# kogdenko/con-gen

Measured on AMD Instinct MI355X. Metric: Gpkts/s + GB/s device-resident checksum, 64B & 1500B batches; %HBM peak, higher is better.
Workload: dtype u16; 1 GPU; 16777216 x 1500 B IPv4+TCP per GPU, dense stride 1500, ip_cksum + tcp_cksum per packet (BASELINE configs[2]; configs[4] at 8 GPUs); packets_per_gpu=16777216, packet_bytes=1500, parallelism=batch-split x1

## Files before the change

### con-gen_amd/csrc/cgck_lane.hip

```cpp
#include "cgck_lane.h"

#include <stdlib.h>
#include <optional>

namespace cgck {


template <bool DESC, bool NT, int S0, bool CLAMP>
__global__ __launch_bounds__(256) void lpp_kernel(KParams p)
{
	const bool raw = p.flags & CGCK_RAW;
	const Sched sc = sched((p.n + 255) / 256, p.contig);
	for (uint64_t it = sc.it; it < sc.end; it += sc.step) {
		const uint64_t k = it * 256 + threadIdx.x;
		const Pkt pk = get_pkt<DESC>(p, k);
		const uint64_t a0 = pk.a0;
		const int len = (int)pk.len, q = (int)(a0 & 15), nch = nchunks(a0, pk.len);
		const uint4 *c0 = reinterpret_cast<const uint4 *>(a0 & ~(uint64_t)15);
		uint4 v[S0];
#pragma unroll
		for (int i = 0; i < S0; ++i)
			v[i] = CLAMP ? ldc<NT>(c0, i, nch, p.zero) : (i < nch ? ld<NT>(c0 + i) : make_uint4(0, 0, 0, 0));
		const bool more = __any(nch > S0);
		uint4 last = make_uint4(0, 0, 0, 0);
		if (CLAMP) {
			if (more)
				last = ldc<NT>(c0, nch - 1, nch, p.zero);
		} else {
			last = nch > S0 ? ld<NT>(c0 + nch - 1) : make_uint4(0, 0, 0, 0);
		}

		uint32_t tot = 0;
#pragma unroll
		for (int i = 0; i < S0; ++i)
			tot = i < nch ? sum4(v[i], tot) : tot;
		Hdr h{};
		if (!raw)
			h = header<S0, NT>(v, c0, nch, q, len, p.flags, pk.ok);
		if (more) {
			for (int t = S0; __any(t < nch - 1); t += 8) {
				uint4 w[8];
#pragma unroll
				for (int i = 0; i < 8; ++i)
					w[i] = t + i < nch - 1 ? ld<NT>(c0 + t + i) : make_uint4(0, 0, 0, 0);
				uint32_t s = 0;
#pragma unroll
				for (int i = 0; i < 8; ++i)
					s = sum4(w[i], s);
				tot = fold16(tot) + fold16(s);
			}
		}
		const bool dw = !__any(((q | len) & 3) != 0);
		if (__any(q != 0))
			tot = fold16(tot) + (0xffffu - fold16(lead_sum(v[0], q, dw)));
		const int e = q + len - 16 * (nch - 1);
		if (more)
			tot = fold16(tot) + fold16(nch > S0 ? sum4(last, 0) - trail_sum(last, e, dw) : 0u);
		if (__any(nch > 0 && nch <= S0 && e != 16)) {
			uint4 lc = make_uint4(0, 0, 0, 0);
#pragma unroll
			for (int i = 0; i < S0; ++i)
				if (i == nch - 1)
					lc = v[i];
			tot = fold16(tot) + (0xffffu - fold16(nch > 0 && nch <= S0 ? trail_sum(lc, e, dw) : 0u));
		}
		if (pk.ok)
			finish(p, k, a0, len, fold16(tot), h);
	}
}

struct Quad {
	uint4 c[4];
};

template <bool NT>
__device__ __forceinline__ void lpa_load(const KParams &p, uint64_t k, bool live, int nch, Quad &q)
{
	k = k < p.n ? k : p.n - 1;
	const uint4 *c0 = live ? reinterpret_cast<const uint4 *>(p.base + k * p.stride + p.l3_off)
			       : reinterpret_cast<const uint4 *>((const uint8_t *)p.zero + (blockIdx.x & 63) * 64);
#pragma unroll
	for (int i = 0; i < 4; ++i)
		q.c[i] = ld<NT>(c0 + (i < nch ? i : nch - 1));
}

template <bool NT, bool STAGE = false, bool IP6 = false>
__device__ __forceinline__ void lpa_reduce(const KParams &p, uint64_t k, int len, int nch, const Quad &q,
					   uint32_t *so = nullptr)
{
	const bool ok = k < p.n;
	if constexpr (IP6) {
		uint32_t T = 0;
#pragma unroll
		for (int i = 0; i < 4; ++i) {
			if (i < nch - 1 || (i == nch - 1 && (len & 15) == 0))
				T = sum4(q.c[i], T);
			else if (i == nch - 1)
				T = msum(q.c[i], 0, 0, len - 16 * i, T);
		}
		const uint32_t h8 = fold16(hsum(q.c[0].y, hsum(q.c[0].x, 0))), nh0 = (q.c[0].y >> 16) & 0xffu;
		const bool plain = len >= 40 && !__any(ok && (v6_is_ext(nh0) || nh0 == 44));
		if (ok) {
			const uint64_t a0 = reinterpret_cast<uint64_t>(p.base) + k * p.stride + p.l3_off;
			uint32_t bl = 0, out = 0;
			if (plain) {
				const int fo = v6_field(nh0);
				if (!(p.flags & CGCK_L4)) {
				} else if (fo >= 0 && 40 + fo + 2 > len) {
					bl = CGCK_BAD_LEN;
				} else {
					const uint32_t L = fold16(ocsub(fold16(T), h8) + (nh0 << 8) + bswap16((uint32_t)(len - 40)));
					out = finish(L) << 16;
				}
			} else {
				out = v6_dense(a0, len, fold16(T), h8, nh0, p.flags, &bl);
			}
			if (STAGE) {
				*so = out;
			} else if (p.out) {
				uint32_t *o = p.out + k;
				asm volatile("global_store_dword %0, %1, off nt" ::"v"(o), "v"(out) : "memory");
			}
			if (p.verdict)
				gbl(p.verdict)[k] = (uint8_t)bl;
		}
		return;
	}
	if (p.flags == (CGCK_IP | CGCK_L4) && (len & 15) == 0 && !__any(ok && (q.c[0].x & 15u) != 5u)) {
		uint32_t T = 0;
#pragma unroll
		for (int i = 0; i < 4; ++i)
			if (i < nch)
				T = sum4(q.c[i], T);
		const uint32_t IPs = fold16(hsum(q.c[1].x, sum4(q.c[0], 0)));
		const uint32_t PS = fold16(hsum(q.c[1].x, hsum(q.c[0].w, 0)));
		const uint32_t proto = (q.c[0].z >> 8) & 0xffu;
		uint32_t L = ocsub(fold16(T), IPs);
		L = fold16(L + PS + (proto << 8) + bswap16((uint32_t)(len - 20)));
		if (ok) {
			const uint32_t out = finish(IPs) | (finish(L) << 16);
			if (STAGE) {
				*so = out;
			} else if (p.out) {
				uint32_t *o = p.out + k;
				asm volatile("global_store_dword %0, %1, off nt" ::"v"(o), "v"(out) : "memory");
			}
			if (p.verdict)
				gbl(p.verdict)[k] = 0;
		}
		return;
	}
	uint4 v[6];
	v[4] = v[5] = make_uint4(0, 0, 0, 0);
#pragma unroll
	for (int i = 0; i < 4; ++i) {
		const int r1 = i < nch - 1 ? 16 : (i == nch - 1 ? len - 16 * i : 0);
		v[i] = make_uint4(q.c[i].x & dmask(0, 0, 0, r1), q.c[i].y & dmask(0, 1, 0, r1),
				  q.c[i].z & dmask(0, 2, 0, r1), q.c[i].w & dmask(0, 3, 0, r1));
	}
	uint32_t tot = 0;
#pragma unroll
	for (int i = 0; i < 4; ++i)
		tot = sum4(v[i], tot);
	const uint64_t a0 = reinterpret_cast<uint64_t>(p.base) + (ok ? k : 0) * p.stride + p.l3_off;
	Hdr h{};
	if (!(p.flags & CGCK_RAW))
		h = header<6, NT>(v, reinterpret_cast<const uint4 *>(a0), nch, 0, len, p.flags, ok);
	if (ok) {
		const Res r = result(p, a0, len, fold16(tot), h);
		if (p.out) {
			if (STAGE) {
				*so = r.out;
			} else {
				uint32_t *o = p.out + k;
				asm volatile("global_store_dword %0, %1, off nt" ::"v"(o), "v"(r.out) : "memory");
			}
		}
		if (p.verdict)
			gbl(p.verdict)[k] = (uint8_t)r.verdict;
	}
}

#define CGCK_LPA_KERNEL lpa_kernel
#define CGCK_LPD_KERNEL lpd_kernel
#define CGCK_LANE_IP6 false
#include "cgck_lane_kernels.inc"
#undef CGCK_LPA_KERNEL
#undef CGCK_LPD_KERNEL
#undef CGCK_LANE_IP6
#define CGCK_LPA_KERNEL lpa6_kernel
#define CGCK_LPD_KERNEL lpd6_kernel
#define CGCK_LANE_IP6 true
#include "cgck_lane_kernels.inc"
#undef CGCK_LPA_KERNEL
#undef CGCK_LPD_KERNEL
#undef CGCK_LANE_IP6


struct SMap {
	uint64_t a0;
	int len, nch;
	int s;
	int st, ns;
	int owner;
	int m;
	bool act;
};

template <bool DESC>
__device__ __forceinline__ SMap smap(const KParams &p, uint64_t cur, uint64_t r1, const DescW &d,
				     uint32_t (&mark)[64])
{
	const int l = threadIdx.x & 63;
	const Pkt pk = decode<DESC>(p, cur + l, r1, d);
	const int nch_l = nchunks(pk.a0, pk.len);
	const uint32_t ns = pk.ok ? (uint32_t)max(1, (nch_l + 7) >> 3) : 0u;
	const uint32_t P = wave_scan_dpp(ns);
	const uint64_t fit = __ballot(pk.ok && P <= 64);
	SMap M;
	M.m = __popcll(fit);
	const int T = M.m ? (int)__builtin_amdgcn_readlane(P, M.m - 1) : 0;
	mark[l] = 0;
	__builtin_amdgcn_wave_barrier();
	asm volatile("" ::: "memory");
	if (l < M.m)
		mark[P - ns] = 1;
	__builtin_amdgcn_wave_barrier();
	asm volatile("" ::: "memory");
	const uint64_t heads = __ballot(mark[l] != 0 && l < T);
	const uint64_t le = l == 63 ? ~0ull : ((2ull << l) - 1);
	const uint64_t below = heads & le, above = heads & ~le;
	M.act = l < T;
	M.owner = below ? __popcll(below) - 1 : 0;
	M.st = below ? 63 - __clzll(below) : 0;
	M.ns = (above ? __ffsll((long long)above) - 1 : T) - M.st;
	M.s = l - M.st;
	M.a0 = shfl64(pk.a0, M.owner);
	M.len = __shfl((int)pk.len, M.owner, 64);
	M.nch = nchunks(M.a0, (uint32_t)M.len);
	return M;
}

template <bool NT>
__device__ __forceinline__ void slot_issue(const KParams &p, const SMap &M, uint4 (&w)[8])
{
	const uint4 *c0 = reinterpret_cast<const uint4 *>(M.a0 & ~(uint64_t)15);
#pragma unroll
	for (int i = 0; i < 8; ++i)
		w[i] = ldc<NT>(c0, 8 * M.s + i, M.nch, p.zero);
}

template <bool NT>
__device__ __forceinline__ void slot_reduce(const KParams &p, uint64_t cur, const SMap &M, uint4 (&w)[8],
					    WaveStage &ws)
{
	const int l = threadIdx.x & 63;
	const bool raw = p.flags & CGCK_RAW;
	const uint64_t a0 = M.a0;
	const int len = M.len, nch = M.nch, s = M.s;
	const int q = (int)(a0 & 15);
	const uint4 *c0 = reinterpret_cast<const uint4 *>(a0 & ~(uint64_t)15);
#pragma unroll
	for (int i = 0; i < 8; ++i)
		asm volatile("" ::"v"(w[i].x), "v"(w[i].y), "v"(w[i].z), "v"(w[i].w));
	if (M.m == 0) {
		const int nsj = (nch + 7) >> 3;
		uint32_t acc = 0;
		Hdr h{};
		for (int wbase = 0; wbase < nsj; wbase += 64) {
			const int sj = wbase + l;
			uint4 (&v)[8] = w;
#pragma unroll
			for (int i = 0; i < 8; ++i)
				v[i] = ldc<NT>(c0, 8 * sj + i, nch, p.zero);
			uint32_t r = 0;
#pragma unroll
			for (int i = 0; i < 8; ++i)
				r = 8 * sj + i < nch ? sum4(v[i], r) : r;
			if (wbase == 0 && !raw)
				h = header<8, NT>(v, c0, nch, q, len, p.flags, l == 0);
			const int j = (nch - 1) - 8 * sj;
			const int e = q + len - 16 * (nch - 1);
			uint32_t corr = 0;
			if (sj == 0 && q != 0)
				corr += lead_sum(v[0], q, false);
			if (j >= 0 && j < 8 && e != 16)
				corr += trail_sum(pick8(v, j), e, false);
			r = fold16(r) + (0xffffu - fold16(corr));
			acc = fold16(acc) + fold16(gsum<64>(r));
		}
		wave_stage_reserve(p, ws, cur, 1);
		if (l == 0)
			wave_stage_put(ws, cur, result(p, a0, len, fold16(acc), h));
		__builtin_amdgcn_s_waitcnt(0);
		return;
	}
	const bool act = M.act;
	uint32_t r = 0;
#pragma unroll
	for (int i = 0; i < 8; ++i)
		r = act && 8 * s + i < nch ? sum4(w[i], r) : r;
	const bool head = act && s == 0;
	Hdr h{};
	if (!raw)
		h = header<8, NT>(w, c0, nch, q, len, p.flags, head);
	const bool dw = !__any(act && ((q | len) & 3) != 0);
	uint32_t corr = 0;
	if (__any(head && q != 0))
		corr = head && q != 0 ? lead_sum(w[0], q, dw) : 0u;
	const int j = (nch - 1) - 8 * s;
	const int e = q + len - 16 * (nch - 1);
	const bool tail = act && nch > 0 && j >= 0 && j < 8 && e != 16;
	if (__any(tail))
		corr += tail ? trail_sum(pick8(w, j), e, dw) : 0u;
	r = fold16(r) + (0xffffu - fold16(corr));
	uint32_t nso = 0;
#pragma unroll
	for (int b = 0; b < 7; ++b)
		nso |= __any(act && ((M.ns >> b) & 1)) ? (1u << b) : 0u;
	const int send = M.st + M.ns;
#pragma unroll
	for (int d = 1; d < 64; d <<= 1) {
		if ((uint32_t)d >= nso)
			break;
		const uint32_t y = __shfl_down(r, d, 64);
		if (l + d < send)
			r += y;
	}
	wave_stage_reserve(p, ws, cur, M.m);
	if (head)
		wave_stage_put(ws, cur + M.owner, result(p, a0, len, fold16(r), h));
}

#if !CGCK_LAB || !defined(CGCK_SLOT2_CHUNK)
#undef CGCK_SLOT2_CHUNK
#define CGCK_SLOT2_CHUNK 0
#endif
template <bool DESC, bool NT>
__global__ __launch_bounds__(256) void slot2_kernel(KParams p)
{
	__shared__ uint32_t mark[4][64];
	__shared__ uint32_t so[4][kWaveStage];
	__shared__ uint8_t sv[4][kWaveStage];
	const int wv = __builtin_amdgcn_readfirstlane(threadIdx.x >> 6), l = threadIdx.x & 63;
	const uint64_t nwaves = (uint64_t)gridDim.x * 4;
	const uint64_t wid = (uint64_t)blockIdx.x * 4 + wv;
#if CGCK_SLOT2_CHUNK
	for (uint64_t ck = wid; ck * CGCK_SLOT2_CHUNK < p.n; ck += nwaves) {
	const uint64_t r0 = ck * CGCK_SLOT2_CHUNK;
	const uint64_t r1 = r0 + CGCK_SLOT2_CHUNK < p.n ? r0 + CGCK_SLOT2_CHUNK : p.n;
#else
	const uint64_t per = (p.n + nwaves - 1) / nwaves;
	const uint64_t r0 = wid * per;
	const uint64_t r1 = r0 + per < p.n ? r0 + per : p.n;
	if (r0 >= r1)
		return;
#endif
	WaveStage ws{so[wv], sv[wv], r0};

	uint64_t curA = r0;
	SMap mA = smap<DESC>(p, curA, r1, load_desc<DESC>(p, curA + l, r1), mark[wv]);
	uint64_t curB = curA + (mA.m ? mA.m : 1);
	DescW dB = load_desc<DESC>(p, curB + l, r1);
	uint4 wA[8], wB[8];
	slot_issue<NT>(p, mA, wA);
	for (;;) {
		const SMap mB = smap<DESC>(p, curB, r1, dB, mark[wv]);
		const uint64_t curC = curB + (mB.m ? mB.m : 1);
		const DescW dC = load_desc<DESC>(p, curC + l, r1);
		slot_issue<NT>(p, mB, wB);
		slot_reduce<NT>(p, curA, mA, wA, ws);
		if (curB >= r1)
			break;
		const SMap mC = smap<DESC>(p, curC, r1, dC, mark[wv]);
		const uint64_t curD = curC + (mC.m ? mC.m : 1);
		dB = load_desc<DESC>(p, curD + l, r1);
		slot_issue<NT>(p, mC, wA);
		slot_reduce<NT>(p, curB, mB, wB, ws);
		if (curC >= r1)
			break;
		curA = curC;
		mA = mC;
		curB = curD;
	}
	wave_stage_flush(p, ws, r1);
#if CGCK_SLOT2_CHUNK
	}
#endif
}

#define CGCK_LPW_KERNEL lpw_kernel
#define CGCK_LPW_IP6 false
#define CGCK_LPW_FILL false
#define CGCK_LPW_MIXED false
#include "cgck_lpw_kernel.inc"
#undef CGCK_LPW_KERNEL
#undef CGCK_LPW_IP6
#undef CGCK_LPW_FILL
#undef CGCK_LPW_MIXED


template <bool DESC, int S0, bool CLAMP>
static hipError_t launch_lpp_t(const KParams &p, int max_blocks, bool nt, hipStream_t st)
{
	const unsigned blocks = grid_blocks(p.n, 256, max_blocks);
	if (nt) {
		CGCK_NOTE_KERNEL("lpp_kernel<%s, true, %d, %s>", tf(DESC), S0, tf(CLAMP));
		hipLaunchKernelGGL((lpp_kernel<DESC, true, S0, CLAMP>), dim3(blocks), dim3(256), 0, st, p);
	} else {
		CGCK_NOTE_KERNEL("lpp_kernel<%s, false, %d, %s>", tf(DESC), S0, tf(CLAMP));
		hipLaunchKernelGGL((lpp_kernel<DESC, false, S0, CLAMP>), dim3(blocks), dim3(256), 0, st, p);
	}
	return hipGetLastError();
}

#if CGCK_LAB
#include "cgck_lane_lab.inc"
#endif

hipError_t launch_lpp(const KParams &p, int num_cus, bool nt, int shape, hipStream_t st)
{
	const int mb = num_cus * 8;
#if CGCK_LAB
	if (const auto lab = launch_lpp_lab(p, mb, nt, shape, st))
		return *lab;
#endif
	return p.desc ? launch_lpp_t<true, 6, false>(p, mb, nt, st) : launch_lpp_t<false, 6, false>(p, mb, nt, st);
}

hipError_t launch_lpd(const KParams &p, int num_cus, hipStream_t st)
{
	static const int wpc = [] {
		const char *e = CGCK_ENV("CGCK_LPD_WPC");
		return e && atoi(e) > 0 ? atoi(e) : 8;
	}();
	const dim3 g(grid_blocks(p.n, 64 * 16, (uint64_t)num_cus * wpc));
	if (p.flags & CGCK_IP6) {
		CGCK_NOTE_KERNEL("lpd6_kernel<2, 32, 2>");
		hipLaunchKernelGGL((lpd6_kernel<2, 32, 2>), g, dim3(64), 2 * 4096 + 32 * 256, st, p);
		return hipGetLastError();
	}
#if CGCK_LAB
	if (const auto lab = launch_lpd_lab(p, g, num_cus, st))
		return *lab;
#endif
	CGCK_NOTE_KERNEL("lpd_kernel<2, 32, 2>");
	hipLaunchKernelGGL((lpd_kernel<2, 32, 2>), g, dim3(64), 2 * 4096 + 32 * 256, st, p);
	return hipGetLastError();
}

hipError_t launch_lpa(const KParams &p, int num_cus, bool nt, hipStream_t st)
{
	static const int bpc = [] {
		const char *e = CGCK_ENV("CGCK_LPA_BPC");
		return e && atoi(e) > 0 ? atoi(e) : 1;
	}();
	static const int depth = [] {
		const char *e = CGCK_ENV("CGCK_LPA_DEPTH");
		const int d = e ? atoi(e) : 0;
		return d >= 2 && d <= 4 ? d : 4;
	}();
	uint64_t want = (p.n + 255) / 256, mb = (uint64_t)num_cus * bpc;
	const dim3 g((unsigned)(want < mb ? want : mb));
	if (p.flags & CGCK_IP6) {
		if (nt) {
			CGCK_NOTE_KERNEL("lpa6_kernel<true, 4>");
			hipLaunchKernelGGL((lpa6_kernel<true, 4>), g, dim3(256), 0, st, p);
		} else {
			CGCK_NOTE_KERNEL("lpa6_kernel<false, 4>");
			hipLaunchKernelGGL((lpa6_kernel<false, 4>), g, dim3(256), 0, st, p);
		}
		return hipGetLastError();
	}
#define CGCK_LPA(D)                                                                            \
	do {                                                                                   \
		if (nt) {                                                                      \
			CGCK_NOTE_KERNEL("lpa_kernel<true, %d>", D);                           \
			hipLaunchKernelGGL((lpa_kernel<true, D>), g, dim3(256), 0, st, p);      \
		} else {                                                                       \
			CGCK_NOTE_KERNEL("lpa_kernel<false, %d>", D);                          \
			hipLaunchKernelGGL((lpa_kernel<false, D>), g, dim3(256), 0, st, p);     \
		}                                                                              \
	} while (0)
	if (depth == 4)
		CGCK_LPA(4);
	else if (depth == 3)
		CGCK_LPA(3);
	else
		CGCK_LPA(2);
#undef CGCK_LPA
	return hipGetLastError();
}

template <bool DESC>
static hipError_t launch_slot2_t(const KParams &p, int max_blocks, bool nt, hipStream_t st)
{
	const unsigned blocks = grid_blocks(p.n, 4 * 64, max_blocks);
	if (nt) {
		CGCK_NOTE_KERNEL("slot2_kernel<%s, true>", tf(DESC));
		hipLaunchKernelGGL((slot2_kernel<DESC, true>), dim3(blocks), dim3(256), 0, st, p);
	} else {
		CGCK_NOTE_KERNEL("slot2_kernel<%s, false>", tf(DESC));
		hipLaunchKernelGGL((slot2_kernel<DESC, false>), dim3(blocks), dim3(256), 0, st, p);
	}
	return hipGetLastError();
}

hipError_t launch_slot2(const KParams &p, int num_cus, bool nt, hipStream_t st)
{
	static const int bpc = [] {
		const char *e = CGCK_ENV("CGCK_BPC");
		return e && atoi(e) > 0 ? atoi(e) : 8;
	}();
	const int mb = num_cus * bpc;
	return p.desc ? launch_slot2_t<true>(p, mb, nt, st) : launch_slot2_t<false>(p, mb, nt, st);
}

hipError_t launch_lpw(const KParams &p, int num_cus, hipStream_t st)
{
	static const int wpc = [] {
		const char *e = CGCK_ENV("CGCK_LPW_WPC");
		return e && atoi(e) > 0 ? atoi(e) : 8;
	}();
	KParams q = p;
	q.contig = 0;
	const LpwShape sh = lpw_shape(p, num_cus, wpc, kLpwSlot);
#if CGCK_LAB
	if (const auto lab = launch_lpw_lab(p, q, sh.grid, sh.lds, num_cus, wpc, st))
		return *lab;
#endif
	if (p.desc) {
		CGCK_NOTE_KERNEL("lpw_kernel<true, %d, false>", kLpwC);
		hipLaunchKernelGGL((lpw_kernel<true, kLpwC, false>), sh.grid, dim3(64), sh.lds, st, q);
	} else {
		CGCK_NOTE_KERNEL("lpw_kernel<false, %d, false>", kLpwC);
		hipLaunchKernelGGL((lpw_kernel<false, kLpwC, false>), sh.grid, dim3(64), sh.lds, st, q);
	}
	return hipGetLastError();
}

}
```

### con-gen_amd/csrc/cgck_lane_kernels.inc

```
template <bool NT, int DEPTH>
__global__ __launch_bounds__(256) void CGCK_LPA_KERNEL(KParams p)
{
	constexpr bool IP6 = CGCK_LANE_IP6;
	const int len = (int)p.ip_len, nch = (len + 15) >> 4;
	const uint64_t NI = (p.n + 255) / 256, S = gridDim.x;
	uint64_t it = blockIdx.x;
	if (it >= NI)
		return;
	Quad Q[DEPTH];
#pragma unroll
	for (int d = 0; d < DEPTH - 1; ++d)
		lpa_load<NT>(p, (it + d * S) * 256 + threadIdx.x, it + d * S < NI, nch, Q[d]);
	for (;;) {
#pragma unroll
		for (int d = 0; d < DEPTH; ++d) {
			const uint64_t ahead = it + (uint64_t)(d + DEPTH - 1) * S;
			lpa_load<NT>(p, ahead * 256 + threadIdx.x, ahead < NI, nch, Q[(d + DEPTH - 1) % DEPTH]);
			lpa_reduce<NT, false, IP6>(p, (it + d * S) * 256 + threadIdx.x, len, nch, Q[d]);
			if (it + (uint64_t)(d + 1) * S >= NI)
				return;
		}
		it += (uint64_t)DEPTH * S;
	}
}

template <int D, int C, int SP>
__global__ __launch_bounds__(64) void CGCK_LPD_KERNEL(KParams p)
{
	constexpr bool IP6 = CGCK_LANE_IP6;
	extern __shared__ __attribute__((aligned(16))) uint8_t smem[];
	const int lane = threadIdx.x;
	const int len = (int)p.ip_len, nch = (len + 15) >> 4;
	const uint32_t lds0 = __builtin_amdgcn_readfirstlane((uint32_t)(uintptr_t)smem);
	uint32_t *so = reinterpret_cast<uint32_t *>(smem + D * 4096);
	const uint8_t *zero = (const uint8_t *)p.zero + (blockIdx.x & 63) * 64;
	const uint64_t base = reinterpret_cast<uint64_t>(p.base) + p.l3_off;
	const uint64_t last_chunk = (base + (p.n - 1) * p.stride + len - 1) & ~(uint64_t)15;
	const uint64_t NS = (p.n + 63) / 64, NC = (NS + C - 1) / C, G = gridDim.x, b = blockIdx.x;
	if (b >= NC)
		return;
	const uint64_t nsteps = (NC - b + G - 1) / G * C;
	auto gstep = [&](uint64_t j) { return (b + (j / C) * G) * C + j % C; };
	const uint32_t span = (uint32_t)(63 * p.stride) + (uint32_t)len;
	auto issue = [&](uint64_t j) {
		const uint64_t gs = gstep(j);
		const uint64_t a = base + gs * 64 * p.stride;
		const uint32_t slot = lds0 + (uint32_t)(j % D) * 4096;
#pragma unroll
		for (int i = 0; i < 4; ++i) {
			const uint32_t at = 1024 * i + 16 * lane;
			const uint64_t src = a + at;
			glds16_nt(j < nsteps && gs < NS && at < span && src <= last_chunk ? reinterpret_cast<const void *>(src)
											  : zero,
				  slot + 1024 * i);
		}
	};
#pragma unroll
	for (int d = 0; d < D - 1; ++d)
		issue(d);
	const int o = lane * (int)p.stride;
	constexpr bool stage = C > 1;
	constexpr bool DEFER = SP >= 3 && C > 1;
	constexpr int policy = SP % 3 == 0 ? kNt : SP % 3 == 1 ? kDefaultPolicy : kSc1;
	u32x4_t held[DEFER ? C / 4 : 1];
	bool pend = false;
	uint64_t pfirst = 0;
	for (uint64_t j = 0; j < nsteps; ++j) {
		issue(j + D - 1);
		if (DEFER && pend) {
			const __amdgpu_buffer_rsrc_t rs = out_rsrc(p.out + pfirst, C * 256);
#pragma unroll
			for (int i = 0; i < (DEFER ? C / 4 : 0); ++i)
				bstore16<policy>(rs, 16 * (i * 64 + lane), held[i]);
			pend = false;
		}
		if (C == 1) {
			if (j + 1 < (uint64_t)D || !p.out)
				asm volatile("s_waitcnt vmcnt(%0)" ::"i"(4 * (D - 1)) : "memory");
			else
				asm volatile("s_waitcnt vmcnt(%0)" ::"i"(5 * (D - 1)) : "memory");
		} else {
			if (stage && j >= (uint64_t)C && (j % C) <= (uint64_t)(DEFER ? D - 1 : D - 2))
				asm volatile("s_waitcnt vmcnt(%0)" ::"i"(4 * (D - 1) + C / 4) : "memory");
			else
				asm volatile("s_waitcnt vmcnt(%0)" ::"i"(4 * (D - 1)) : "memory");
		}
		__builtin_amdgcn_s_barrier();
		const uint8_t *sl = smem + (uint32_t)(j % D) * 4096;
		Quad q;
#pragma unroll
		for (int i = 0; i < 4; ++i)
			q.c[i] = *reinterpret_cast<const uint4 *>(sl + o + 16 * (i < nch ? i : nch - 1));
		asm volatile("s_waitcnt lgkmcnt(0)" ::: "memory");
		const uint64_t k = gstep(j) * 64 + lane;
		if (stage)
			lpa_reduce<false, true, IP6>(p, k, len, nch, q, so + (j % C) * 64 + lane);
		else
			lpa_reduce<false, false, IP6>(p, k, len, nch, q);
		if (stage && (j + 1) % C == 0 && p.contig != 2) {
			const uint64_t first = (b + (j / C) * G) * C * 64;
			asm volatile("s_waitcnt lgkmcnt(0)" ::: "memory");
			if (DEFER && first + C * 64 <= p.n && j + 1 < nsteps) {
				const u32x4_t *s4 = reinterpret_cast<const u32x4_t *>(so);
#pragma unroll
				for (int i = 0; i < (DEFER ? C / 4 : 0); ++i)
					held[i] = s4[i * 64 + lane];
				asm volatile("s_waitcnt lgkmcnt(0)" ::: "memory");
				pend = true;
				pfirst = first;
			} else if (first + C * 64 <= p.n) {
				const uint4 *s4 = reinterpret_cast<const uint4 *>(so);
				const __amdgpu_buffer_rsrc_t rs = out_rsrc(p.out + first, C * 256);
#pragma unroll
				for (int i = 0; i < C / 4; ++i) {
					const uint4 w = s4[i * 64 + lane];
					bstore16<policy>(rs, 16 * (i * 64 + lane), u32x4_t{w.x, w.y, w.z, w.w});
				}
			} else {
				for (int i = lane; i < C * 64; i += 64)
					if (first + i < p.n)
						gbl(p.out)[first + i] = so[i];
				asm volatile("s_waitcnt vmcnt(0)" ::: "memory");
			}
		}
	}
	asm volatile("s_waitcnt vmcnt(0)" ::: "memory");
}
```

Before: 4.523 Gpkt/s.

## Add specialized hot loop to LDS-staged checksum kernel with inline-asm batched loads

Splits the LPD kernel main loop into a hot phase covering full, in-bounds steps and a generic tail phase. The hot phase uses compile-time window counts and a fast-path flag, strength-reduced address and packet-index counters, and a single inline-asm block that issues the four global_load_lds_dwordx4 through m0 increments. It also precomputes LDS read indices and makes bounds checks unnecessary via a FULL template flag. The aim is to cut per-step scalar and vector ALU overhead (divisions, bounds checks, address math) so the kernel stays bandwidth-bound, at the cost of more code variants and fragile hand-written asm.

Measured after the change: 4.521 Gpkt/s. Within noise of the previous version (-0.1%).

```diff
diff --git a/con-gen_amd/csrc/cgck_lane.hip b/con-gen_amd/csrc/cgck_lane.hip
--- a/con-gen_amd/csrc/cgck_lane.hip
+++ b/con-gen_amd/csrc/cgck_lane.hip
@@ -84,11 +84,11 @@
 		q.c[i] = ld<NT>(c0 + (i < nch ? i : nch - 1));
 }
 
-template <bool NT, bool STAGE = false, bool IP6 = false>
+template <bool NT, bool STAGE = false, bool IP6 = false, int FAST = -1, bool FULL = false>
 __device__ __forceinline__ void lpa_reduce(const KParams &p, uint64_t k, int len, int nch, const Quad &q,
-					   uint32_t *so = nullptr)
-{
-	const bool ok = k < p.n;
+					   uint32_t *so = nullptr, uint64_t a0full = 0)
+{
+	const bool ok = FULL || k < p.n;
 	if constexpr (IP6) {
 		uint32_t T = 0;
 #pragma unroll
@@ -101,7 +101,7 @@
 		const uint32_t h8 = fold16(hsum(q.c[0].y, hsum(q.c[0].x, 0))), nh0 = (q.c[0].y >> 16) & 0xffu;
 		const bool plain = len >= 40 && !__any(ok && (v6_is_ext(nh0) || nh0 == 44));
 		if (ok) {
-			const uint64_t a0 = reinterpret_cast<uint64_t>(p.base) + k * p.stride + p.l3_off;
+			const uint64_t a0 = FULL ? a0full : reinterpret_cast<uint64_t>(p.base) + k * p.stride + p.l3_off;
 			uint32_t bl = 0, out = 0;
 			if (plain) {
 				const int fo = v6_field(nh0);
@@ -126,12 +126,13 @@
 		}
 		return;
 	}
-	if (p.flags == (CGCK_IP | CGCK_L4) && (len & 15) == 0 && !__any(ok && (q.c[0].x & 15u) != 5u)) {
+	if (FAST != 0 && (FAST == 1 || (p.flags == (CGCK_IP | CGCK_L4) && (len & 15) == 0)) &&
+	    !__any(ok && (q.c[0].x & 15u) != 5u)) {
 		uint32_t T = 0;
 #pragma unroll
 		for (int i = 0; i < 4; ++i)
 			if (i < nch)
-				T = sum4(q.c[i], T);
+				T += sum4(q.c[i], 0);
 		const uint32_t IPs = fold16(hsum(q.c[1].x, sum4(q.c[0], 0)));
 		const uint32_t PS = fold16(hsum(q.c[1].x, hsum(q.c[0].w, 0)));
 		const uint32_t proto = (q.c[0].z >> 8) & 0xffu;
@@ -162,7 +163,7 @@
 #pragma unroll
 	for (int i = 0; i < 4; ++i)
 		tot = sum4(v[i], tot);
-	const uint64_t a0 = reinterpret_cast<uint64_t>(p.base) + (ok ? k : 0) * p.stride + p.l3_off;
+	const uint64_t a0 = FULL ? a0full : reinterpret_cast<uint64_t>(p.base) + (ok ? k : 0) * p.stride + p.l3_off;
 	Hdr h{};
 	if (!(p.flags & CGCK_RAW))
 		h = header<6, NT>(v, reinterpret_cast<const uint4 *>(a0), nch, 0, len, p.flags, ok);
@@ -180,6 +181,45 @@
 			gbl(p.verdict)[k] = (uint8_t)r.verdict;
 	}
 }
+
+#define CGCK_LP_OPEN "s_mov_b32 %[k], m0\n\ts_mov_b32 m0, %[slot]\n\ts_nop 2\n\t"
+#define CGCK_LP_NEXT "s_add_u32 m0, m0, 0x400\n\ts_nop 0\n\t"
+#define CGCK_LP_W(i) "global_load_lds_dwordx4 %[o" #i "], %[a] nt\n\t"
+#define CGCK_LP_P "global_load_lds_dwordx4 %[pa], off nt\n\t"
+#define CGCK_LP_Z "global_load_lds_dwordx4 %[vz], %[z] nt\n\t"
+#define CGCK_LP_ASM(d0, d1, d2, d3)                                                                     \
+	asm volatile(CGCK_LP_OPEN d0 CGCK_LP_NEXT d1 CGCK_LP_NEXT d2 CGCK_LP_NEXT d3 "s_mov_b32 m0, %[k]"   \
+		     : [k] "=&s"(keep)                                                                   \
+		     : [slot] "s"(slot), [a] "s"(a), [o0] "v"(off[0]), [o1] "v"(off[1]), [o2] "v"(off[2]), \
+		       [o3] "v"(off[3]), [pa] "v"(pa), [vz] "v"(vz), [z] "s"(z)                           \
+		     : "memory", "scc")
+template <int NW>
+__device__ __forceinline__ void lpd_issue_full(uint64_t a, uint32_t slot, const uint32_t (&off)[4], const void *pa,
+						const void *z, uint32_t vz)
+{
+	static_assert(NW >= 0 && NW <= 4, "a step is at most 4 KiB");
+	uint32_t keep;
+	if constexpr (NW == 4)
+		CGCK_LP_ASM(CGCK_LP_W(0), CGCK_LP_W(1), CGCK_LP_W(2), CGCK_LP_W(3));
+	else if constexpr (NW == 3)
+		CGCK_LP_ASM(CGCK_LP_W(0), CGCK_LP_W(1), CGCK_LP_W(2), CGCK_LP_P);
+	else if constexpr (NW == 2)
+		CGCK_LP_ASM(CGCK_LP_W(0), CGCK_LP_W(1), CGCK_LP_P, CGCK_LP_Z);
+	else if constexpr (NW == 1)
+		CGCK_LP_ASM(CGCK_LP_W(0), CGCK_LP_P, CGCK_LP_Z, CGCK_LP_Z);
+	else
+		CGCK_LP_ASM(CGCK_LP_P, CGCK_LP_Z, CGCK_LP_Z, CGCK_LP_Z);
+}
+#undef CGCK_LP_ASM
+#undef CGCK_LP_Z
+#undef CGCK_LP_P
+#undef CGCK_LP_W
+#undef CGCK_LP_NEXT
+#undef CGCK_LP_OPEN
+
+#ifndef CGCK_LPD_REFILL_EARLY
+#define CGCK_LPD_REFILL_EARLY 0
+#endif
 
 #define CGCK_LPA_KERNEL lpa_kernel
 #define CGCK_LPD_KERNEL lpd_kernel
diff --git a/con-gen_amd/csrc/cgck_lane_kernels.inc b/con-gen_amd/csrc/cgck_lane_kernels.inc
--- a/con-gen_amd/csrc/cgck_lane_kernels.inc
+++ b/con-gen_amd/csrc/cgck_lane_kernels.inc
@@ -55,18 +55,62 @@
 				  slot + 1024 * i);
 		}
 	};
-#pragma unroll
-	for (int d = 0; d < D - 1; ++d)
-		issue(d);
 	const int o = lane * (int)p.stride;
 	constexpr bool stage = C > 1;
 	constexpr bool DEFER = SP >= 3 && C > 1;
 	constexpr int policy = SP % 3 == 0 ? kNt : SP % 3 == 1 ? kDefaultPolicy : kSc1;
+	constexpr bool EARLY = CGCK_LPD_REFILL_EARLY && !DEFER && C > 1;
+	constexpr int AHEAD = EARLY ? D : D - 1;
+
+	uint32_t rd[4];
+#pragma unroll
+	for (int i = 0; i < 4; ++i)
+		rd[i] = opaque((uint32_t)((o >> 4) + (i < nch ? i : nch - 1)));
+	const uint32_t nw = span >> 10;
+	uint32_t off[4];
+#pragma unroll
+	for (int i = 0; i < 4; ++i)
+		off[i] = opaque(1024u * i + 16u * lane);
+	const uint32_t poff = 1024 * nw + 16 * lane;
+	const uint32_t pmask = opaque(poff < span ? ~0u : 0u);
+	const uint32_t vz = opaque(0u);
+	const uint32_t ns32 = (uint32_t)nsteps;
+	const uint32_t klast = ns32 / C - 1;
+	const uint64_t lrem = (p.n - (b + (uint64_t)klast * G) * C * 64) / 64;
+	const uint32_t jfull = klast * C + (lrem < (uint64_t)C ? (uint32_t)lrem : (uint32_t)C);
+	const uint64_t step64 = 64 * p.stride, kjump = (G * C - (C - 1)) * 64, cjump = kjump * p.stride;
+	uint64_t ia = base + gstep(AHEAD) * step64;
+	uint64_t ra = base + b * C * step64, ks = b * C * 64;
+	uint32_t slot_off = 0, islot = (AHEAD % D) * 4096;
+
+#pragma unroll
+	for (int d = 0; d < AHEAD; ++d)
+		issue(d);
 	u32x4_t held[DEFER ? C / 4 : 1];
 	bool pend = false;
 	uint64_t pfirst = 0;
-	for (uint64_t j = 0; j < nsteps; ++j) {
-		issue(j + D - 1);
+	auto step = [&](uint32_t j, auto nwc, auto fastc) __attribute__((always_inline)) {
+		constexpr int NW = decltype(nwc)::value, FAST = decltype(fastc)::value;
+		constexpr bool HOT = NW >= 0;
+		auto refill = [&]() __attribute__((always_inline)) {
+			if constexpr (HOT) {
+				const void *pa = zero;
+				if constexpr (NW < 4) {
+					const uint64_t pl = ia + poff;
+					const uint64_t zl = reinterpret_cast<uint64_t>(zero);
+					pa = reinterpret_cast<const void *>(
+						(uint64_t)pick(pmask, (uint32_t)pl, (uint32_t)zl) |
+						(uint64_t)pick(pmask, (uint32_t)(pl >> 32), (uint32_t)(zl >> 32)) << 32);
+				}
+				lpd_issue_full<NW>(ia, lds0 + islot, off, pa, zero, vz);
+				ia += ((j + AHEAD + 1) % C) == 0 ? cjump : step64;
+				islot = islot + 4096 == D * 4096 ? 0 : islot + 4096;
+			} else {
+				issue((uint64_t)j + AHEAD);
+			}
+		};
+		if (!EARLY)
+			refill();
 		if (DEFER && pend) {
 			const __amdgpu_buffer_rsrc_t rs = out_rsrc(p.out + pfirst, C * 256);
 #pragma unroll
@@ -75,32 +119,38 @@
 			pend = false;
 		}
 		if (C == 1) {
-			if (j + 1 < (uint64_t)D || !p.out)
+			if (j + 1 < (uint32_t)D || !p.out)
 				asm volatile("s_waitcnt vmcnt(%0)" ::"i"(4 * (D - 1)) : "memory");
 			else
 				asm volatile("s_waitcnt vmcnt(%0)" ::"i"(5 * (D - 1)) : "memory");
 		} else {
-			if (stage && j >= (uint64_t)C && (j % C) <= (uint64_t)(DEFER ? D - 1 : D - 2))
+			if (stage && j >= (uint32_t)C && (j % C) <= (uint32_t)(DEFER || EARLY ? D - 1 : D - 2))
 				asm volatile("s_waitcnt vmcnt(%0)" ::"i"(4 * (D - 1) + C / 4) : "memory");
 			else
 				asm volatile("s_waitcnt vmcnt(%0)" ::"i"(4 * (D - 1)) : "memory");
 		}
 		__builtin_amdgcn_s_barrier();
-		const uint8_t *sl = smem + (uint32_t)(j % D) * 4096;
+		const u32x4_t *sl = reinterpret_cast<const u32x4_t *>(smem + slot_off);
 		Quad q;
 #pragma unroll
-		for (int i = 0; i < 4; ++i)
-			q.c[i] = *reinterpret_cast<const uint4 *>(sl + o + 16 * (i < nch ? i : nch - 1));
+		for (int i = 0; i < 4; ++i) {
+			const u32x4_t w = sl[rd[i]];
+			q.c[i] = make_uint4(w.x, w.y, w.z, w.w);
+		}
 		asm volatile("s_waitcnt lgkmcnt(0)" ::: "memory");
-		const uint64_t k = gstep(j) * 64 + lane;
+		if (EARLY)
+			refill();
+		const uint64_t k = (HOT ? ks : gstep(j) * 64) + lane;
+		[[maybe_unused]] const uint64_t a0 = (ra + (uint32_t)o) & ~(uint64_t)15;
 		if (stage)
-			lpa_reduce<false, true, IP6>(p, k, len, nch, q, so + (j % C) * 64 + lane);
+			lpa_reduce<false, true, IP6, FAST, HOT>(p, k, len, nch, q, so + (j % C) * 64 + lane, a0);
 		else
-			lpa_reduce<false, false, IP6>(p, k, len, nch, q);
+			lpa_reduce<false, false, IP6, FAST, HOT>(p, k, len, nch, q, nullptr, a0);
 		if (stage && (j + 1) % C == 0 && p.contig != 2) {
-			const uint64_t first = (b + (j / C) * G) * C * 64;
+			const uint64_t first = HOT ? ks - (C - 1) * 64 : (b + (uint64_t)(j / C) * G) * C * 64;
+			const bool whole = HOT || first + C * 64 <= p.n;
 			asm volatile("s_waitcnt lgkmcnt(0)" ::: "memory");
-			if (DEFER && first + C * 64 <= p.n && j + 1 < nsteps) {
+			if (DEFER && whole && (uint64_t)j + 1 < nsteps) {
 				const u32x4_t *s4 = reinterpret_cast<const u32x4_t *>(so);
 #pragma unroll
 				for (int i = 0; i < (DEFER ? C / 4 : 0); ++i)
@@ -108,7 +158,7 @@
 				asm volatile("s_waitcnt lgkmcnt(0)" ::: "memory");
 				pend = true;
 				pfirst = first;
-			} else if (first + C * 64 <= p.n) {
+			} else if (whole) {
 				const uint4 *s4 = reinterpret_cast<const uint4 *>(so);
 				const __amdgpu_buffer_rsrc_t rs = out_rsrc(p.out + first, C * 256);
 #pragma unroll
@@ -123,6 +173,38 @@
 				asm volatile("s_waitcnt vmcnt(0)" ::: "memory");
 			}
 		}
+		if constexpr (HOT) {
+			const bool ce = (j + 1) % C == 0;
+			ra += ce ? cjump : step64;
+			ks += ce ? kjump : 64;
+		}
+		slot_off = slot_off + 4096 == D * 4096 ? 0 : slot_off + 4096;
+	};
+	constexpr bool ALLNW = D == 2 && C == 32;
+	const bool fast = !IP6 && p.flags == (CGCK_IP | CGCK_L4) && (len & 15) == 0;
+	const uint32_t jhot = jfull > (uint32_t)AHEAD && (ALLNW || nw == 4) ? jfull - AHEAD : 0;
+	uint32_t j = 0;
+	auto hot = [&](auto nwc) __attribute__((always_inline)) {
+		if (IP6 || !fast) {
+			for (; j < jhot; ++j)
+				step(j, nwc, std::integral_constant<int, 0>{});
+		} else {
+			for (; j < jhot; ++j)
+				step(j, nwc, std::integral_constant<int, 1>{});
+		}
+	};
+	if (ALLNW) {
+		switch (nw) {
+		case 4: hot(std::integral_constant<int, 4>{}); break;
+		case 3: hot(std::integral_constant<int, 3>{}); break;
+		case 2: hot(std::integral_constant<int, 2>{}); break;
+		case 1: hot(std::integral_constant<int, 1>{}); break;
+		default: hot(std::integral_constant<int, 0>{}); break;
+		}
+	} else {
+		hot(std::integral_constant<int, 4>{});
 	}
+	for (; j < ns32; ++j)
+		step(j, std::integral_constant<int, -1>{}, std::integral_constant<int, -1>{});
 	asm volatile("s_waitcnt vmcnt(0)" ::: "memory");
 }
```
